# HKUST-Aerial-Robotics/FUEL

Hardware: NVIDIA H100
Metric: replans_per_sec (higher is better)
Workload: dtype f64 (cost/gradient), i32+f32 (ESDF), u8 (frontier)

## Files before the change

### fuel_b200/csrc/frontier.cu

```cuda
#include "common.cuh"

#include <cooperative_groups.h>

#include <algorithm>
#include <vector>

namespace cg = cooperative_groups;

namespace {

constexpr int NONE = 0x7fffffff;

struct FParams {
  int dom_lo[3], dom_n[3];
  int s_lo[3], s_hi[3];
  int z_min_idx;
  int cluster_min;
  double size_xy;
  float leaf, leaf_inv;
};

__device__ __forceinline__ int tri_at(const Geom& g, const uint8_t* __restrict__ occ, int x, int y,
                                      int z) {
  if (x < 0 || y < 0 || z < 0 || x >= g.nx || y >= g.ny || z >= g.nz) return -1;
// ... 1036 lines not shown
  int* c_final;
  int* ccur;
  int* cnext;
};

__global__ void stat_accum_kernel(Geom g, const int* __restrict__ k_addr, const int* __restrict__ k_cl,
                                  const ClusterMeta* __restrict__ meta, ClusterStat* st, LevelCtl ctl) {
  if (*ctl.n_new == 0) return;
  stat_accum_item(g, k_addr, k_cl, meta, st, *ctl.K, blockIdx.x * blockDim.x + threadIdx.x);
}

__global__ void downsample_kernel(Geom g, FParams fp, const int* __restrict__ k_addr,
                                  const int* __restrict__ k_cl, const int* __restrict__ cellidx,
                                  const ClusterMeta* __restrict__ meta, ClusterStat* st,
                                  float* __restrict__ k_cent, int* __restrict__ k_leaf, LevelCtl ctl) {
  if (*ctl.n_new == 0) return;
  downsample_item<true>(g, fp, k_addr, k_cl, cellidx, meta, st, k_cent, k_leaf, *ctl.K, blockIdx.x * blockDim.x + threadIdx.x);
}

__global__ void cov_kernel(Geom g, const int* __restrict__ k_cl, const int* __restrict__ k_leaf,
                           const float* __restrict__ k_cent, const ClusterMeta* __restrict__ meta,
                           ClusterStat* st, LevelCtl ctl) {
  if (*ctl.n_new == 0) return;
  cov_item<true>(g, k_cl, k_leaf, k_cent, meta, st, *ctl.K, blockIdx.x * blockDim.x + threadIdx.x);
}

__global__ void pca_kernel(Geom g, ClusterMeta* meta, const ClusterStat* __restrict__ st, LevelCtl ctl) {
  if (*ctl.n_new == 0) return;
  const int c = blockIdx.x * blockDim.x + threadIdx.x;
  mean_item(g, meta, st, *ctl.ccur, c);
  pca_item(meta, st, *ctl.ccur, c);
}

__global__ void side_count_kernel(Geom g, const int* __restrict__ k_addr, const int* __restrict__ k_cl,
                                  const ClusterMeta* __restrict__ meta, ClusterStat* st, LevelCtl ctl) {
  if (*ctl.n_new == 0) return;
  side_count_item(g, k_addr, k_cl, meta, st, *ctl.K, blockIdx.x * blockDim.x + threadIdx.x);
}

__global__ void __launch_bounds__(1024) split_alloc_kernel(ClusterMeta* meta, const ClusterStat* __restrict__ st,
                                                           LevelCtl ctl) {
  if (*ctl.n_new == 0) return;
  const int C = *ctl.ccur;
  __shared__ int made;
  split_alloc(meta, st, C, &made);
  __syncthreads();
  if (threadIdx.x == 0) {
    *ctl.cnext = C + made;
    *ctl.c_final = C + made;
    *ctl.n_new = made;
  }
}

__global__ void relabel_kernel(Geom g, const int* __restrict__ k_addr, int* __restrict__ k_cl,
                               const ClusterMeta* __restrict__ meta, LevelCtl ctl) {
  if (*ctl.n_new == 0) return;
  relabel_item(g, k_addr, k_cl, meta, *ctl.K, *ctl.ccur, blockIdx.x * blockDim.x + threadIdx.x);
}

__global__ void next_level_kernel(ClusterMeta* meta, ClusterStat* st, LevelCtl ctl) {
  if (*ctl.n_new == 0) return;
  const int c = blockIdx.x * blockDim.x + threadIdx.x;
  clear_do_split_item(meta, *ctl.ccur, c);
  stat_reset_item(st, meta, *ctl.cnext, c);
}

__global__ void init_meta_kernel(ClusterMeta* meta, ClusterStat* st, LevelCtl ctl) {
  const int R = *ctl.R;
  const int c = blockIdx.x * blockDim.x + threadIdx.x;
  init_meta_item(meta, R, c);
  stat_reset_item(st, meta, R, c);
  if (c == 0) {
    *ctl.ccur = R;
    *ctl.c_final = R;
    *ctl.n_new = (R > 0 && *ctl.K > 0) ? 1 : 0;
  }
}


constexpr int SMALL_CTAS = 8;
constexpr int SMALL_CAP = 32768;
constexpr int SMALL_CCAP = 8192;
constexpr int RES_K0 = 12288, RES_C0 = 256;


__device__ __forceinline__ void mark_chunk_item(const int* __restrict__ seed, const int* __restrict__ csize, int cluster_min,
                                                int* __restrict__ root_mask, int* __restrict__ kept_mask, int n, int i) {
  bool kept = false, root = false;
  if (i < n) {
    const int s = seed[i];
    kept = s != NONE && csize[s] > cluster_min;
    root = kept && s == i;
  }
  const unsigned mk = __ballot_sync(0xffffffffu, kept), mr = __ballot_sync(0xffffffffu, root);
  if ((i & 31) == 0 && i < n) {
    kept_mask[i >> 5] = (int)mk;
    root_mask[i >> 5] = (int)mr;
  }
}
__device__ void chunk_scan_small(const int* __restrict__ root_mask, const int* __restrict__ kept_mask,
                                 int* __restrict__ root_off, int* __restrict__ kept_off, int nchunk,
                                 int* __restrict__ tot_root, int* __restrict__ tot_kept) {
  __shared__ unsigned wtot2[32];
  const int t = threadIdx.x, lane = t & 31, w = t >> 5;
  const unsigned v = t < nchunk ? ((unsigned)__popc((unsigned)root_mask[t]) << 16) + (unsigned)__popc((unsigned)kept_mask[t]) : 0u;
  unsigned inc = v;
#pragma unroll
  for (int o = 1; o < 32; o <<= 1) {
    const unsigned u = __shfl_up_sync(0xffffffffu, inc, o);
    if (lane >= o) inc += u;
  }
  if (lane == 31) wtot2[w] = inc;
  __syncthreads();
  if (w == 0) {
    const unsigned x = wtot2[lane];
    unsigned xi = x;
#pragma unroll
    for (int o = 1; o < 32; o <<= 1) {
      const unsigned u = __shfl_up_sync(0xffffffffu, xi, o);
      if (lane >= o) xi += u;
    }
    wtot2[lane] = xi - x;
    if (lane == 31) {
      *tot_root = (int)(xi >> 16);
      *tot_kept = (int)(xi & 0xffffu);
    }
  }
  __syncthreads();
  if (t < nchunk) {
    const unsigned ex = wtot2[w] + inc - v;
    root_off[t] = (int)(ex >> 16);
    kept_off[t] = (int)(ex & 0xffffu);
  }
}
__device__ __forceinline__ void gather_chunk_item(const int* __restrict__ cell_addr, const int* __restrict__ seed,
                                                  const int* __restrict__ kept_mask, const int* __restrict__ kept_off,
                                                  const int* __restrict__ root_mask, const int* __restrict__ root_off,
                                                  int* __restrict__ k_addr, int* __restrict__ k_cl,
                                                  int* __restrict__ cellidx, int n, int i) {
  if (i >= n) return;
  const unsigned mk = (unsigned)kept_mask[i >> 5];
  const int a = cell_addr[i];
  if ((mk >> (i & 31)) & 1u) {
    const int k = kept_off[i >> 5] + __popc(mk & ((1u << (i & 31)) - 1u));
    const int s = seed[i];
    k_addr[k] = a;
    k_cl[k] = root_off[s >> 5] + __popc((unsigned)root_mask[s >> 5] & ((1u << (s & 31)) - 1u));
    cellidx[a] = k;
  } else {
    cellidx[a] = -1;
  }
}

struct SmallBufs {
  int *cell_addr, *parent, *claim, *csize, *seed, *is_root, *is_kept, *root_rank, *kept_off;
  uint8_t* cell_cls;
  int *k_addr, *k_cl, *k_leaf;
  float* k_cent;
  ClusterMeta* meta;
  ClusterStat* stat;
  int* counters;
  int* r_counters;
  ClusterMeta* r_meta;
  ClusterStat* r_stat;
  int *r_addr, *r_cl, *r_leaf;
  float* r_cent;
  int r_K, r_C;
};

__global__ void __cluster_dims__(SMALL_CTAS, 1, 1) __launch_bounds__(1024) cluster_small_kernel(Geom g, FParams fp, int8_t* __restrict__ flag,
                                                             int* __restrict__ cellidx, SmallBufs b) {
  cg::cluster_group cluster = cg::this_cluster();
  const int rank = (int)cluster.block_rank();
  const int tid = (((int)threadIdx.x >> 5) * SMALL_CTAS + rank) * 32 + ((int)threadIdx.x & 31);
  constexpr int NT = 1024 * SMALL_CTAS;
  const int n = b.counters[0];
#ifdef FUEL_PROF
  long long* prof = (long long*)(b.counters + 8);
  int pi = 0;
#define STAMP() do { if (tid == 0) { long long t_; asm volatile("mov.u64 %0, %%globaltimer;" : "=l"(t_)); prof[pi++] = t_; } } while (0)
#else
#define STAMP() do {} while (0)
#endif
  STAMP();
  if (n > SMALL_CAP) {
    if (tid == 0) {
      b.counters[4] = 1;
      b.r_counters[0] = n;
      b.r_counters[4] = 1;
    }
    return;
  }
#define FOR_ITEMS(i, N) for (int i = tid; i - tid < (N); i += NT)
  FOR_ITEMS(i, n) init_parent_item(b.parent, b.claim, b.csize, n, i);
  cluster.sync();
  STAMP();
  FOR_ITEMS(i, n) union_item(g, b.cell_addr, b.cell_cls, cellidx, b.parent, n, i);
  cluster.sync();
  STAMP();
  FOR_ITEMS(i, n) flatten_item(b.parent, b.cell_cls, n, i);
  cluster.sync();
  STAMP();
  FOR_ITEMS(i, n) claim_item(g, fp, b.cell_addr, b.cell_cls, cellidx, b.parent, b.claim, n, i);
  cluster.sync();
  STAMP();
  FOR_ITEMS(i, n) assign_item(b.cell_addr, b.cell_cls, b.parent, b.claim, b.seed, b.csize, flag, n, i);
  cluster.sync();
  STAMP();
  FOR_ITEMS(i, n) mark_chunk_item(b.seed, b.csize, fp.cluster_min, b.is_root, b.is_kept, n, i);
  cluster.sync();
  STAMP();
  if (rank == 0) chunk_scan_small(b.is_root, b.is_kept, b.root_rank, b.kept_off, (n + 31) >> 5, b.counters + 1, b.counters + 2);
  cluster.sync();
  STAMP();
  const int R = b.counters[1], K = b.counters[2];
  int C = R;
  int status = 0;
  if (R > 0 && K > 0) {
    FOR_ITEMS(i, n) gather_chunk_item(b.cell_addr, b.seed, b.is_kept, b.kept_off, b.is_root, b.root_rank, b.k_addr, b.k_cl,
                                      cellidx, n, i);
    FOR_ITEMS(c, R) {
      init_meta_item(b.meta, R, c);
      stat_reset_item(b.stat, b.meta, R, c);
    }
    cluster.sync();
    STAMP();
    for (int level = 0; level < 40; ++level) {
      if (2 * C > SMALL_CCAP) {
        status = 2;
        break;
      }
      FOR_ITEMS(k, K) stat_accum_item(g, b.k_addr, b.k_cl, b.meta, b.stat, K, k);
      cluster.sync();
      STAMP();
      FOR_ITEMS(c, C) mean_item(g, b.meta, b.stat, C, c);
      FOR_ITEMS(k, K) downsample_item<true>(g, fp, b.k_addr, b.k_cl, cellidx, b.meta, b.stat, b.k_cent, b.k_leaf, K, k);
      cluster.sync();
      STAMP();
      FOR_ITEMS(k, K) cov_item(g, b.k_cl, b.k_leaf, b.k_cent, b.meta, b.stat, K, k);
      cluster.sync();
      STAMP();
      FOR_ITEMS(c, C) pca_item(b.meta, b.stat, C, c);
      cluster.sync();
      STAMP();
      FOR_ITEMS(k, K) side_count_item(g, b.k_addr, b.k_cl, b.meta, b.stat, K, k);
      cluster.sync();
      STAMP();
      if (rank == 0) split_alloc(b.meta, b.stat, C, b.counters + 3);
      cluster.sync();
      STAMP();
      FOR_ITEMS(k, K) relabel_item(g, b.k_addr, b.k_cl, b.meta, K, C, k);
      cluster.sync();
      STAMP();
      const int n_new = b.counters[3];
      if (n_new == 0) break;
      FOR_ITEMS(c, C) clear_do_split_item(b.meta, C, c);
      C += n_new;
      FOR_ITEMS(c, C) stat_reset_item(b.stat, b.meta, C, c);
      cluster.sync();
      STAMP();
    }
  }
  FOR_ITEMS(i, n) reset_cellidx_item(b.cell_addr, cellidx, n, i);
  if (status == 0 && R > 0 && K > 0) {
    const int kp = min(K, b.r_K), cp = min(C, b.r_C);
    FOR_ITEMS(k, kp) {
      if (k < kp) {
        b.r_addr[k] = b.k_addr[k];
        b.r_cl[k] = b.k_cl[k];
        b.r_leaf[k] = b.k_leaf[k];
        b.r_cent[3 * k] = b.k_cent[3 * k];
        b.r_cent[3 * k + 1] = b.k_cent[3 * k + 1];
        b.r_cent[3 * k + 2] = b.k_cent[3 * k + 2];
      }
    }
    FOR_ITEMS(c, cp) {
      if (c < cp) {
        b.r_meta[c] = b.meta[c];
        b.r_stat[c] = b.stat[c];
      }
    }
  }
  if (tid == 0) {
    b.counters[4] = status;
    b.counters[5] = C;
    const int out[8] = { n, R, K, b.counters[3], status, C, b.counters[6], b.counters[7] };
#pragma unroll
    for (int j = 0; j < 8; ++j) b.r_counters[j] = out[j];
  }
#undef FOR_ITEMS
}

__global__ void is_changed_kernel(Geom g, const uint8_t* __restrict__ occ, const int* __restrict__ offs,
                                  const int* __restrict__ addr, uint8_t* __restrict__ changed, int* __restrict__ counts,
                                  int m) {
  const int c = blockIdx.x;
  if (c >= m) return;
  __shared__ int cnt;
  if (threadIdx.x == 0) cnt = 0;
  __syncthreads();
  int mine = 0;
  for (int i = offs[c] + threadIdx.x; i < offs[c + 1]; i += blockDim.x) {
    int x, y, z;
    addr_to_idx(g, addr[i], x, y, z);
    if (!frontier_pred(g, occ, x, y, z)) ++mine;
  }
  if (mine) atomicAdd(&cnt, mine);
  __syncthreads();
  if (threadIdx.x == 0) {
    if (changed) changed[c] = (uint8_t)(cnt > 0);
    if (counts) counts[c] = cnt;
  }
}

template <typename T>
struct DevBuf {
  T* p = nullptr;
  size_t cap = 0;
  int ensure(size_t n) {
    if (n <= cap) return 0;
    if (p) cudaFree(p);
    p = nullptr;
    cap = 0;
    size_t want = n + n / 4 + 1024;
    if (cudaMalloc(&p, want * sizeof(T)) != cudaSuccess) return FUELGPU_ENOMEM;
    cap = want;
    return 0;
  }
  int grow_preserve(size_t n, size_t keep, cudaStream_t s) {
    if (n <= cap) return 0;
    T* np = nullptr;
    size_t want = n + n / 2 + 1024;
    if (cudaMalloc(&np, want * sizeof(T)) != cudaSuccess) return FUELGPU_ENOMEM;
    if (p && keep) {
      cudaMemcpyAsync(np, p, keep * sizeof(T), cudaMemcpyDeviceToDevice, s);
      cudaStreamSynchronize(s);
    }
    if (p) cudaFree(p);
    p = np;
    cap = want;
    return 0;
  }
  void release() {
    if (p) cudaFree(p);
    p = nullptr;
    cap = 0;
  }
};

}

struct SweepPlan {
  bool words = false;
  unsigned nb = 0;
  size_t nmask = 0;
  int64_t ndom = 0;
  WordGeom wg;
};

struct HostView {
  const int *addr, *cl, *leaf;
  const float* cent;
  const ClusterMeta* meta;
  const ClusterStat* stat;
};

struct FrontierState {
  int* cellidx = nullptr;
  DevBuf<uint32_t> maskE, maskS;
  DevBuf<int> blockcnt, blockoff, scan_tot, scan_off;
  DevBuf<int> cell_addr, parent, claim, csize, seed, is_root, is_kept, root_rank, kept_off;
  DevBuf<uint8_t> cell_cls;
  DevBuf<int> k_addr, k_cl, k_leaf;
  DevBuf<float> k_cent;
  DevBuf<ClusterStat> stat;
  DevBuf<ClusterMeta> meta;
  DevBuf<char> res;
  bool small_ready = false;
  bool pend_active = false, pend_empty = true;
  FParams pend_fp;
  SweepPlan pend_plan;
  HostView pend_hv;
  cudaStream_t stream = nullptr;
  cudaEvent_t ev_in = nullptr;
  cudaEvent_t ev_out = nullptr;
  bool ev_out_valid = false;
  char* h_pin = nullptr;
  size_t h_pin_bytes = 0;
  int* d_counters = nullptr;
  std::vector<int32_t> h_cell_off, h_cell_addr, h_filt_off;
  std::vector<double> h_filtered, h_avg, h_bmin, h_bmax;
  int cell_order = FUELGPU_CELLS_BY_ADDRESS;
  float last_leaf = 0.f;
};

cudaStream_t frontier_stream_raw(FuelMap* m) { return m->fs->stream; }
cudaStream_t frontier_stream(FuelMap* m) {
  FrontierState* f = m->fs;
  cudaEventRecord(f->ev_in, m->stream);
  cudaStreamWaitEvent(f->stream, f->ev_in, 0);
  return f->stream;
}

int frontier_set_cell_order(FuelMap* m, int order) {
  if (order != FUELGPU_CELLS_BY_ADDRESS && order != FUELGPU_CELLS_BFS)
    return fuel_fail(m, FUELGPU_EINVAL, "unknown cell order");
  m->fs->cell_order = order;
  return 0;
}

void frontier_order_writer(FuelMap* m) {
  FrontierState* f = m->fs;
  if (f && f->ev_out_valid) cudaStreamWaitEvent(m->stream, f->ev_out, 0);
}

int frontier_state_create(FuelMap* m) {
  m->fs = new FrontierState();
  FUEL_CUDA(m, cudaStreamCreateWithFlags(&m->fs->stream, cudaStreamNonBlocking));
  FUEL_CUDA(m, cudaEventCreateWithFlags(&m->fs->ev_in, cudaEventDisableTiming));
  FUEL_CUDA(m, cudaEventCreateWithFlags(&m->fs->ev_out, cudaEventDisableTiming));
  FUEL_CUDA(m, cudaMalloc(&m->fs->cellidx, sizeof(int) * m->nvox));
  FUEL_CUDA(m, cudaMemsetAsync(m->fs->cellidx, 0xff, sizeof(int) * m->nvox, m->stream));
  FUEL_CUDA(m, cudaMalloc(&m->fs->d_counters, sizeof(int) * 8 + sizeof(long long) * 256));
  FUEL_CUDA(m, cudaMemsetAsync(m->fs->d_counters, 0, sizeof(int) * 8 + sizeof(long long) * 256, m->stream));
  return 0;
}

void frontier_state_destroy(FuelMap* m) {
  if (!m->fs) return;
  FrontierState* f = m->fs;
  if (f->cellidx) cudaFree(f->cellidx);
  if (f->d_counters) cudaFree(f->d_counters);
  if (f->h_pin) cudaFreeHost(f->h_pin);
  if (f->stream) {
    cudaStreamSynchronize(f->stream);
    cudaStreamDestroy(f->stream);
  }
  if (f->ev_in) cudaEventDestroy(f->ev_in);
  if (f->ev_out) cudaEventDestroy(f->ev_out);
  f->maskE.release(); f->maskS.release(); f->blockcnt.release(); f->blockoff.release();
  f->scan_tot.release(); f->scan_off.release();
  f->cell_addr.release(); f->parent.release(); f->claim.release(); f->csize.release();
  f->seed.release(); f->is_root.release(); f->is_kept.release(); f->root_rank.release();
  f->kept_off.release(); f->cell_cls.release(); f->k_addr.release(); f->k_cl.release();
  f->k_leaf.release(); f->k_cent.release(); f->stat.release(); f->meta.release(); f->res.release();
  delete f;
  m->fs = nullptr;
}

#define ENSURE(buf, n)                                         \
  do {                                                         \
    if ((buf).ensure(n)) return fuel_fail(m, FUELGPU_ENOMEM, "frontier: device allocation failed"); \
  } while (0)

static inline unsigned nblk(int64_t n, int b) { return (unsigned)((n + b - 1) / b); }

static int scan_ints(FuelMap* m, const int* in, int* out, int n, int* total) {
  FrontierState* f = m->fs;
  cudaStream_t s = m->fs->stream;
  if (n <= 4096) {
    scan_kernel<<<1, 1024, 0, s>>>(in, out, n, total);
    FUEL_LAUNCHES(m, 1);
    return 0;
  }
  const int nchunk = (n + 1023) / 1024;
  if (f->scan_tot.ensure(nchunk) || f->scan_off.ensure(nchunk))
    return fuel_fail(m, FUELGPU_ENOMEM, "frontier: device allocation failed");
  scan_chunks_kernel<<<nchunk, 1024, 0, s>>>(in, out, n, f->scan_tot.p);
  scan_kernel<<<1, 1024, 0, s>>>(f->scan_tot.p, f->scan_off.p, nchunk, total);
  scan_add_kernel<<<nchunk, 1024, 0, s>>>(out, n, f->scan_off.p);
  FUEL_LAUNCHES(m, 3);
  return 0;
}

static SweepPlan sweep_plan(const Geom& g, const FParams& fp) {
  SweepPlan pl;
  pl.ndom = (int64_t)fp.dom_n[0] * fp.dom_n[1] * fp.dom_n[2];
  pl.words = (g.nz % 32) == 0 && pl.ndom > 0;
  if (pl.words) {
    const int z0 = fp.dom_lo[2], z1 = fp.dom_lo[2] + fp.dom_n[2] - 1;
    pl.wg.wz0 = z0 >> 5;
    pl.wg.NW = (z1 >> 5) - pl.wg.wz0 + 1;
    pl.wg.nwords = (int64_t)fp.dom_n[0] * fp.dom_n[1] * pl.wg.NW;
    pl.nb = nblk(pl.wg.nwords, WORD_BLOCK);
    pl.nmask = (size_t)pl.nb * WORD_BLOCK;
  } else {
    pl.nb = nblk(pl.ndom, CLS_BLOCK);
    pl.nmask = (size_t)pl.nb * (CLS_BLOCK / 32);
  }
  return pl;
}

static int sweep_classify(FuelMap* m, const FParams& fp, const SweepPlan& pl, cudaStream_t s) {
  FrontierState* f = m->fs;
  ENSURE(f->maskE, pl.nmask);
  ENSURE(f->maskS, pl.nmask);
  ENSURE(f->blockcnt, pl.nb);
  ENSURE(f->blockoff, pl.nb);
  if (pl.words)
    classify_words_kernel<<<pl.nb, WORD_BLOCK, 0, s>>>(m->g, fp, pl.wg, m->occ, m->flag, f->maskE.p, f->maskS.p,
                                                       f->blockcnt.p);
  else
    classify_kernel<<<pl.nb, CLS_BLOCK, 0, s>>>(m->g, fp, m->occ, m->flag, f->maskE.p, f->maskS.p, f->blockcnt.p,
                                                pl.ndom);
  FUEL_LAUNCHES(m, 1);
  if (scan_ints(m, f->blockcnt.p, f->blockoff.p, (int)pl.nb, f->d_counters + 0)) return FUELGPU_ENOMEM;
  return 0;
}

static void sweep_compact(FuelMap* m, const FParams& fp, const SweepPlan& pl, int* cellidx, int cap, cudaStream_t s) {
  FrontierState* f = m->fs;
  if (pl.words)
    compact_words_kernel<<<pl.nb, WORD_BLOCK, 0, s>>>(m->g, fp, pl.wg, f->maskE.p, f->maskS.p, f->blockoff.p,
                                                      f->cell_addr.p, f->cell_cls.p, cellidx, cap);
  else
    compact_kernel<<<pl.nb, CLS_BLOCK, 0, s>>>(m->g, fp, f->maskE.p, f->maskS.p, f->blockoff.p, f->cell_addr.p,
                                               f->cell_cls.p, cellidx, pl.ndom, cap);
  FUEL_LAUNCHES(m, 1);
}

static size_t view_bytes(int K, int C) {
  return (size_t)K * (3 * sizeof(int) + 3 * sizeof(float)) + (size_t)C * (sizeof(ClusterMeta) + sizeof(ClusterStat)) + 64;
}

static int ensure_pin(FuelMap* m, size_t bytes) {
  FrontierState* f = m->fs;
  if (bytes <= f->h_pin_bytes) return 0;
  if (f->h_pin) cudaFreeHost(f->h_pin);
  f->h_pin = nullptr;
  f->h_pin_bytes = 0;
  FUEL_CUDA(m, cudaMallocHost((void**)&f->h_pin, bytes));
  f->h_pin_bytes = bytes;
  return 0;
}

struct ResultLayout {
  size_t meta, stat, addr, cl, leaf, cent, bytes;
};
static ResultLayout result_layout(int K, int C) {
  ResultLayout l;
  size_t p = 0;
  auto put = [&](size_t bytes) {
// ... 135 lines not shown
      for (int i = 0; i < cn; ++i) {
        int ijk[3];
        for (int a = 0; a < 3; ++a) ijk[a] = (int)(floorf(pf[(size_t)3 * i + a] * inv) - (float)minb[a]);
        lk[i] = std::make_pair(ijk[0] + ijk[1] * divb[0] + ijk[2] * divb[0] * divb[1], i);
      }
      std::sort(lk.begin(), lk.end());
      int nf = 0;
      for (int i = 0; i < cn;) {
        int j = i;
        float acc[3] = { 0.f, 0.f, 0.f };
        while (j < cn && lk[j].first == lk[i].first) {
          for (int a = 0; a < 3; ++a) acc[a] += pf[(size_t)3 * lk[j].second + a];
          ++j;
        }
        const float cntf = (float)(j - i);
        for (int a = 0; a < 3; ++a) new_filtered.push_back((double)(acc[a] / cntf));
        ++nf;
        i = j;
      }
      new_filt_off[r + 1] = new_filt_off[r] + nf;
    }
    r0 = r1;
  }
  f->h_filt_off.swap(new_filt_off);
  f->h_filtered.swap(new_filtered);
}

static int frontier_marshal(FuelMap* m, int K, int C, int32_t* n_clusters, int32_t* n_cells,
                            int32_t* n_filtered) {
  int rc = ensure_pin(m, view_bytes(K, C));
  if (rc) return rc;
  HostView hv;
  rc = enqueue_download(m, K, C, m->fs->h_pin, &hv);
  if (rc) return rc;
  FUEL_CUDA(m, cudaStreamSynchronize(m->fs->stream));
  return frontier_build_csr(m, K, C, hv, n_clusters, n_cells, n_filtered);
}

static int frontier_build_csr(FuelMap* m, int K, int C, const HostView& hv, int32_t* n_clusters,
                              int32_t* n_cells, int32_t* n_filtered) {
  FrontierState* f = m->fs;
  const Geom& g = m->g;
  const int* h_addr = hv.addr;
  const int* h_cl = hv.cl;
  const int* h_leaf = hv.leaf;
  const float* h_cent = hv.cent;
  const ClusterMeta* h_meta = hv.meta;
  const ClusterStat* h_stat = hv.stat;
  std::vector<int> order(C);
  for (int c = 0; c < C; ++c) order[c] = c;
  std::sort(order.begin(), order.end(), [&](int a, int b) {
    if (h_meta[a].root != h_meta[b].root) return h_meta[a].root < h_meta[b].root;
    return h_meta[a].path < h_meta[b].path;
  });
  std::vector<int> rank(C);
  for (int i = 0; i < C; ++i) rank[order[i]] = i;

  f->h_cell_off.assign(C + 1, 0);
  f->h_filt_off.assign(C + 1, 0);
  for (int k = 0; k < K; ++k) {
    f->h_cell_off[rank[h_cl[k]] + 1]++;
    if (h_leaf[k] >= 0) f->h_filt_off[rank[h_cl[k]] + 1]++;
  }
  for (int c = 0; c < C; ++c) {
    f->h_cell_off[c + 1] += f->h_cell_off[c];
    f->h_filt_off[c + 1] += f->h_filt_off[c];
  }
  f->h_cell_addr.resize(K);
  const int NF = f->h_filt_off[C];
  std::vector<std::pair<int, int>> filt_keys(NF);
  {
    std::vector<int> cur(f->h_cell_off.begin(), f->h_cell_off.end() - 1);
    std::vector<int> curf(f->h_filt_off.begin(), f->h_filt_off.end() - 1);
    for (int k = 0; k < K; ++k) {
      const int r = rank[h_cl[k]];
      f->h_cell_addr[cur[r]++] = h_addr[k];
      if (h_leaf[k] >= 0) filt_keys[curf[r]++] = std::make_pair(h_leaf[k], k);
    }
  }
  f->h_filtered.resize((size_t)3 * NF);
  for (int c = 0; c < C; ++c) {
    std::sort(filt_keys.begin() + f->h_filt_off[c], filt_keys.begin() + f->h_filt_off[c + 1]);
    for (int i = f->h_filt_off[c]; i < f->h_filt_off[c + 1]; ++i) {
      const int k = filt_keys[i].second;
      for (int a = 0; a < 3; ++a) f->h_filtered[(size_t)3 * i + a] = (double)h_cent[(size_t)3 * k + a];
    }
  }
  f->h_avg.resize((size_t)3 * C);
  f->h_bmin.resize((size_t)3 * C);
  f->h_bmax.resize((size_t)3 * C);
  for (int c = 0; c < C; ++c) {
    const int r = rank[c];
    for (int a = 0; a < 3; ++a) {
      f->h_avg[(size_t)3 * r + a] = h_meta[c].mean[a];
      f->h_bmin[(size_t)3 * r + a] = (h_stat[c].lo[a] + 0.5) * g.res + g.origin[a];
      f->h_bmax[(size_t)3 * r + a] = (h_stat[c].hi[a] + 0.5) * g.res + g.origin[a];
    }
  }
  *n_clusters = C;
  *n_cells = K;
  *n_filtered = NF;
  if (f->cell_order == FUELGPU_CELLS_BFS) {
    std::vector<int> out_root(C);
    for (int c = 0; c < C; ++c) out_root[rank[c]] = h_meta[c].root;
    frontier_apply_bfs_order(m, out_root);
    *n_filtered = f->h_filt_off[C];
  }
  return 0;
}

static int frontier_cluster_large(FuelMap* m, const FParams& fp, int n_cand, int32_t* n_clusters, int32_t* n_cells,
                                  int32_t* n_filtered);

static void frontier_make_params(FuelMap* m, const double umin[3], const double umax[3], const FuelFrontierParams* p,
                                 FParams* out) {
  FrontierState* f = m->fs;
  const Geom& g = m->g;
  const int nmax[3] = { g.nx, g.ny, g.nz };
  FParams fp;
  const double infl[3] = { 1, 1, 0.5 };
  for (int k = 0; k < 3; ++k) {
    double lo = umin[k] - infl[k], hi = umax[k] + infl[k];
    lo = lo > g.box_mind[k] ? lo : g.box_mind[k];
    hi = hi < g.box_maxd[k] ? hi : g.box_maxd[k];
    int ilo = (int)floor((lo - g.origin[k]) * g.res_inv);
    int ihi = (int)floor((hi - g.origin[k]) * g.res_inv);
    fp.s_lo[k] = ilo < 0 ? 0 : ilo;
    fp.s_hi[k] = ihi > nmax[k] - 1 ? nmax[k] - 1 : ihi;
    int dlo = g.box_min[k] < fp.s_lo[k] ? g.box_min[k] : fp.s_lo[k];
    int dhi = g.box_max[k] > fp.s_hi[k] ? g.box_max[k] : fp.s_hi[k];
    dlo = dlo < 0 ? 0 : dlo;
    dhi = dhi > nmax[k] - 1 ? nmax[k] - 1 : dhi;
    fp.dom_lo[k] = dlo;
    fp.dom_n[k] = dhi - dlo + 1;
    if (fp.dom_n[k] <= 0) {
      fp.dom_n[k] = 0;
    }
  }
  {
    int zi = 0;
    while (zi < g.nz && ((zi + 0.5) * g.res + g.origin[2]) < p->min_z) ++zi;
    fp.z_min_idx = zi;
  }
  fp.cluster_min = p->cluster_min;
  fp.size_xy = p->cluster_size_xy;
  fp.leaf = (float)(g.res * p->down_sample);
  f->last_leaf = fp.leaf;
  fp.leaf_inv = 1.0f / fp.leaf;
  f->pend_fp = fp;
  *out = fp;
}

static void frontier_clear_results(FrontierState* f) {
  f->h_cell_off.assign(1, 0);
  f->h_cell_addr.clear();
  f->h_filt_off.assign(1, 0);
  f->h_filtered.clear();
  f->h_avg.clear();
  f->h_bmin.clear();
  f->h_bmax.clear();
  f->pend_active = false;
  f->pend_empty = true;
}

int frontier_search_begin_impl(FuelMap* m, const double umin[3], const double umax[3],
                               const FuelFrontierParams* p) {
  FrontierState* f = m->fs;
  const Geom& g = m->g;
  cudaStream_t s = m->fs->stream;
  FParams fp;
  frontier_make_params(m, umin, umax, p, &fp);

  f->h_cell_off.assign(1, 0);
  f->h_cell_addr.clear();
  f->h_filt_off.assign(1, 0);
  f->h_filtered.clear();
  f->h_avg.clear();
  f->h_bmin.clear();
  f->h_bmax.clear();
  f->pend_active = false;
  f->pend_empty = true;

  const SweepPlan pl = sweep_plan(g, fp);
  if (pl.ndom <= 0) return 0;
  f->pend_empty = false;
  {
    const int rc = sweep_classify(m, fp, pl, s);
    if (rc) return rc;
  }
  {
    ENSURE(f->cell_addr, SMALL_CAP); ENSURE(f->cell_cls, SMALL_CAP); ENSURE(f->parent, SMALL_CAP);
    ENSURE(f->claim, SMALL_CAP); ENSURE(f->csize, SMALL_CAP); ENSURE(f->seed, SMALL_CAP);
    ENSURE(f->is_root, SMALL_CAP); ENSURE(f->is_kept, SMALL_CAP); ENSURE(f->root_rank, SMALL_CAP);
    ENSURE(f->kept_off, SMALL_CAP); ENSURE(f->k_addr, SMALL_CAP); ENSURE(f->k_cl, SMALL_CAP);
    ENSURE(f->k_leaf, SMALL_CAP); ENSURE(f->k_cent, (size_t)3 * SMALL_CAP);
    ENSURE(f->meta, SMALL_CCAP); ENSURE(f->stat, SMALL_CCAP);
    const ResultLayout rl = result_layout(RES_K0, RES_C0);
    ENSURE(f->res, 64 + rl.bytes);
    sweep_compact(m, fp, pl, f->cellidx, SMALL_CAP, s);
    SmallBufs sb;
    sb.cell_addr = f->cell_addr.p; sb.parent = f->parent.p; sb.claim = f->claim.p; sb.csize = f->csize.p;
    sb.seed = f->seed.p; sb.is_root = f->is_root.p; sb.is_kept = f->is_kept.p; sb.root_rank = f->root_rank.p;
    sb.kept_off = f->kept_off.p; sb.cell_cls = f->cell_cls.p; sb.k_addr = f->k_addr.p; sb.k_cl = f->k_cl.p;
    sb.k_leaf = f->k_leaf.p; sb.k_cent = f->k_cent.p; sb.meta = f->meta.p; sb.stat = f->stat.p;
    sb.counters = f->d_counters;
    {
      char* rb = f->res.p + 64;
      sb.r_counters = (int*)f->res.p;
      sb.r_meta = (ClusterMeta*)(rb + rl.meta); sb.r_stat = (ClusterStat*)(rb + rl.stat);
      sb.r_addr = (int*)(rb + rl.addr); sb.r_cl = (int*)(rb + rl.cl); sb.r_leaf = (int*)(rb + rl.leaf);
      sb.r_cent = (float*)(rb + rl.cent);
      sb.r_K = RES_K0;
      sb.r_C = RES_C0;
    }
    cluster_small_kernel<<<SMALL_CTAS, 1024, 0, s>>>(g, fp, m->flag, f->cellidx, sb);
    FUEL_LAUNCHES(m, 1);
    int rc0 = ensure_pin(m, 64 + rl.bytes);
    if (rc0) return rc0;
    FUEL_CUDA(m, cudaMemcpyAsync(f->h_pin, f->res.p, 64 + rl.bytes, cudaMemcpyDeviceToHost, s));
    result_view(rl, f->h_pin + 64, &f->pend_hv);
    f->pend_fp = fp;
    f->pend_plan = pl;
    f->pend_active = true;
  }
  cudaEventRecord(f->ev_out, f->stream);
  f->ev_out_valid = true;
  return 0;
}

int frontier_search_end_impl(FuelMap* m, int32_t* n_clusters, int32_t* n_cells, int32_t* n_filtered) {
  FrontierState* f = m->fs;
  const Geom& g = m->g;
  cudaStream_t s = m->fs->stream;
  *n_clusters = *n_cells = *n_filtered = 0;
  if (f->pend_empty || !f->pend_active) {
    f->pend_active = false;
    return 0;
  }
  f->pend_active = false;
  const FParams fp = f->pend_fp;
  const SweepPlan pl = f->pend_plan;
  int n_cand = 0;
  {
    const int* cnt = (const int*)f->h_pin;
    HostView& hv = f->pend_hv;
    FUEL_CUDA(m, cudaStreamSynchronize(s));
    n_cand = cnt[0];
    if (n_cand == 0) return 0;
    if (cnt[4] == 0) {
      const int R = cnt[1], K = cnt[2], C = cnt[5];
      if (R == 0 || K == 0) return 0;
      if (K <= RES_K0 && C <= RES_C0) return frontier_build_csr(m, K, C, hv, n_clusters, n_cells, n_filtered);
      return frontier_marshal(m, K, C, n_clusters, n_cells, n_filtered);
    }
    if (cnt[4] == 1) {
      reset_cellidx_kernel<<<nblk(SMALL_CAP, 256), 256, 0, s>>>(f->cell_addr.p, f->cellidx, SMALL_CAP);
      FUEL_LAUNCHES(m, 1);
    }
  }

  ENSURE(f->cell_addr, n_cand); ENSURE(f->cell_cls, n_cand); ENSURE(f->parent, n_cand);
  ENSURE(f->claim, n_cand); ENSURE(f->csize, n_cand); ENSURE(f->seed, n_cand);
  ENSURE(f->is_root, n_cand); ENSURE(f->is_kept, n_cand); ENSURE(f->root_rank, n_cand);
  ENSURE(f->kept_off, n_cand);

  sweep_compact(m, fp, pl, f->cellidx, n_cand, s);
  return frontier_cluster_large(m, fp, n_cand, n_clusters, n_cells, n_filtered);
}

static int frontier_cluster_large(FuelMap* m, const FParams& fp, int n_cand, int32_t* n_clusters, int32_t* n_cells,
                                  int32_t* n_filtered) {
  FrontierState* f = m->fs;
  const Geom& g = m->g;
  cudaStream_t s = m->fs->stream;
  ENSURE(f->parent, n_cand);
  ENSURE(f->claim, n_cand); ENSURE(f->csize, n_cand); ENSURE(f->seed, n_cand);
  ENSURE(f->is_root, n_cand); ENSURE(f->is_kept, n_cand); ENSURE(f->root_rank, n_cand);
  ENSURE(f->kept_off, n_cand);
  ENSURE(f->k_addr, n_cand); ENSURE(f->k_cl, n_cand); ENSURE(f->k_leaf, n_cand); ENSURE(f->k_cent, (size_t)3 * n_cand);
  ENSURE(f->meta, (size_t)n_cand + 1024);
  ENSURE(f->stat, (size_t)n_cand + 1024);
  const unsigned cb = nblk(n_cand, 256);
  init_parent_kernel<<<cb, 256, 0, s>>>(f->parent.p, f->claim.p, f->csize.p, n_cand);
  union_kernel<<<cb, 256, 0, s>>>(g, f->cell_addr.p, f->cell_cls.p, f->cellidx, f->parent.p, n_cand);
  flatten_kernel<<<cb, 256, 0, s>>>(f->parent.p, f->cell_cls.p, n_cand);
  claim_kernel<<<cb, 256, 0, s>>>(g, fp, f->cell_addr.p, f->cell_cls.p, f->cellidx, f->parent.p, f->claim.p, n_cand);
  assign_kernel<<<cb, 256, 0, s>>>(f->cell_addr.p, f->cell_cls.p, f->parent.p, f->claim.p, f->seed.p,
                                   f->csize.p, m->flag, n_cand);
  mark_kernel<<<cb, 256, 0, s>>>(f->seed.p, f->csize.p, fp.cluster_min, f->is_root.p, f->is_kept.p, n_cand);
  FUEL_LAUNCHES(m, 6);
  if (scan_ints(m, f->is_root.p, f->root_rank.p, n_cand, f->d_counters + 1)) return FUELGPU_ENOMEM;
  if (scan_ints(m, f->is_kept.p, f->kept_off.p, n_cand, f->d_counters + 2)) return FUELGPU_ENOMEM;
  gather_kept_kernel<<<cb, 256, 0, s>>>(f->cell_addr.p, f->seed.p, f->is_kept.p, f->kept_off.p,
                                        f->root_rank.p, f->k_addr.p, f->k_cl.p, f->cellidx, n_cand);
  FUEL_LAUNCHES(m, 1);

  LevelCtl ctl;
  ctl.R = f->d_counters + 1;
  ctl.K = f->d_counters + 2;
  ctl.n_new = f->d_counters + 3;
  ctl.c_final = f->d_counters + 5;
  ctl.ccur = f->d_counters + 6;
  ctl.cnext = f->d_counters + 7;
  const int64_t r_ub = n_cand / ((fp.cluster_min > 0 ? fp.cluster_min : 0) + 1) + 1;
  init_meta_kernel<<<nblk(r_ub, 256), 256, 0, s>>>(f->meta.p, f->stat.p, ctl);
  FUEL_LAUNCHES(m, 1);
  int cnt[8] = { 0, 0, 0, 0, 0, 0, 0, 0 };
  constexpr int LEVELS_PER_BATCH = 12, MAX_LEVELS = 36;
  auto c_bound = [&](int level) -> int64_t {
    const int64_t c = level < 24 ? (r_ub << level) : (int64_t)n_cand;
    return c > n_cand ? (int64_t)n_cand : c;
  };
  for (int level = 0; level < MAX_LEVELS; ++level) {
    const unsigned ccb = nblk(c_bound(level), 256);
    stat_accum_kernel<<<cb, 256, 0, s>>>(g, f->k_addr.p, f->k_cl.p, f->meta.p, f->stat.p, ctl);
    downsample_kernel<<<cb, 256, 0, s>>>(g, fp, f->k_addr.p, f->k_cl.p, f->cellidx, f->meta.p, f->stat.p,
                                         f->k_cent.p, f->k_leaf.p, ctl);
    cov_kernel<<<cb, 256, 0, s>>>(g, f->k_cl.p, f->k_leaf.p, f->k_cent.p, f->meta.p, f->stat.p, ctl);
    pca_kernel<<<ccb, 256, 0, s>>>(g, f->meta.p, f->stat.p, ctl);
    side_count_kernel<<<cb, 256, 0, s>>>(g, f->k_addr.p, f->k_cl.p, f->meta.p, f->stat.p, ctl);
    split_alloc_kernel<<<1, 1024, 0, s>>>(f->meta.p, f->stat.p, ctl);
    relabel_kernel<<<cb, 256, 0, s>>>(g, f->k_addr.p, f->k_cl.p, f->meta.p, ctl);
    next_level_kernel<<<nblk(c_bound(level + 1), 256), 256, 0, s>>>(f->meta.p, f->stat.p, ctl);
    FUEL_LAUNCHES(m, 8);
    int* t = ctl.ccur;
    ctl.ccur = ctl.cnext;
    ctl.cnext = t;
    if ((level + 1) % LEVELS_PER_BATCH == 0 || level + 1 == MAX_LEVELS) {
      FUEL_CUDA(m, cudaMemcpyAsync(cnt, f->d_counters, sizeof(int) * 8, cudaMemcpyDeviceToHost, s));
      FUEL_CUDA(m, cudaStreamSynchronize(s));
      if (cnt[3] == 0) break;
    }
  }
  reset_cellidx_kernel<<<cb, 256, 0, s>>>(f->cell_addr.p, f->cellidx, n_cand);
  FUEL_LAUNCHES(m, 1);
  FUEL_CUDA(m, cudaGetLastError());
  const int R = cnt[1], K = cnt[2], C = cnt[5];
  if (R == 0 || K == 0) return 0;
  return frontier_marshal(m, K, C, n_clusters, n_cells, n_filtered);
}


__global__ void set_cellidx_kernel(const int* __restrict__ cell_addr, int* __restrict__ cellidx, int n) {
  const int i = blockIdx.x * blockDim.x + threadIdx.x;
  if (i < n) cellidx[cell_addr[i]] = i;
}

int frontier_candidates_impl(FuelMap* m, const double umin[3], const double umax[3], const FuelFrontierParams* p, int z_lo,
                             int z_hi, int32_t* n_out) {
  FrontierState* f = m->fs;
  const Geom& g = m->g;
  cudaStream_t s = frontier_stream(m);
  FParams fp;
  frontier_make_params(m, umin, umax, p, &fp);
  *n_out = 0;
  const int dz0 = fp.dom_lo[2] > z_lo ? fp.dom_lo[2] : z_lo;
  const int dz1 = (fp.dom_lo[2] + fp.dom_n[2] - 1) < z_hi ? (fp.dom_lo[2] + fp.dom_n[2] - 1) : z_hi;
  if (dz1 < dz0) return 0;
  fp.dom_lo[2] = dz0;
  fp.dom_n[2] = dz1 - dz0 + 1;
  const SweepPlan pl = sweep_plan(g, fp);
  if (pl.ndom <= 0) return 0;
  {
    const int rc = sweep_classify(m, fp, pl, s);
    if (rc) return rc;
  }
  int n = 0;
  FUEL_CUDA(m, cudaMemcpyAsync(&n, f->d_counters, sizeof(int), cudaMemcpyDeviceToHost, s));
  FUEL_CUDA(m, cudaStreamSynchronize(s));
  if (n > 0) {
    ENSURE(f->cell_addr, n);
    ENSURE(f->cell_cls, n);
    sweep_compact(m, fp, pl, nullptr, n, s);
    FUEL_CUDA(m, cudaGetLastError());
  }
  *n_out = n;
  return 0;
}

int frontier_candidates_fetch_impl(FuelMap* m, int32_t n, int32_t* addr, uint8_t* cls) {
  FrontierState* f = m->fs;
  if (n <= 0) return 0;
  cudaStream_t s = f->stream;
  FUEL_CUDA(m, cudaMemcpyAsync(addr, f->cell_addr.p, sizeof(int) * n, cudaMemcpyDeviceToHost, s));
  FUEL_CUDA(m, cudaMemcpyAsync(cls, f->cell_cls.p, n, cudaMemcpyDeviceToHost, s));
  FUEL_CUDA(m, cudaStreamSynchronize(s));
  return 0;
}

int frontier_search_from_candidates_impl(FuelMap* m, const double umin[3], const double umax[3], const FuelFrontierParams* p,
                                         int32_t n, const int32_t* addr, const uint8_t* cls, int32_t* n_clusters,
                                         int32_t* n_cells, int32_t* n_filtered) {
  FrontierState* f = m->fs;
  cudaStream_t s = frontier_stream(m);
  FParams fp;
  frontier_make_params(m, umin, umax, p, &fp);
  frontier_clear_results(f);
  *n_clusters = *n_cells = *n_filtered = 0;
  if (n <= 0) return 0;
  for (int i = 1; i < n; ++i)
    if (addr[i] <= addr[i - 1]) return fuel_fail(m, FUELGPU_EINVAL, "candidate addresses must be strictly ascending");
  if (addr[0] < 0 || (int64_t)addr[n - 1] >= m->nvox) return fuel_fail(m, FUELGPU_EINVAL, "candidate address outside the map");
  ENSURE(f->cell_addr, n);
  ENSURE(f->cell_cls, n);
  FUEL_CUDA(m, cudaMemcpyAsync(f->cell_addr.p, addr, sizeof(int) * n, cudaMemcpyHostToDevice, s));
  FUEL_CUDA(m, cudaMemcpyAsync(f->cell_cls.p, cls, n, cudaMemcpyHostToDevice, s));
  set_cellidx_kernel<<<nblk(n, 256), 256, 0, s>>>(f->cell_addr.p, f->cellidx, n);
  FUEL_LAUNCHES(m, 1);
  FUEL_CUDA(m, cudaMemcpyAsync(f->d_counters, &n, sizeof(int), cudaMemcpyHostToDevice, s));
  const int rc = frontier_cluster_large(m, fp, n, n_clusters, n_cells, n_filtered);
  cudaEventRecord(f->ev_out, f->stream);
  f->ev_out_valid = true;
  return rc;
}

int frontier_search_impl(FuelMap* m, const double umin[3], const double umax[3],
                         const FuelFrontierParams* p, int32_t* n_clusters, int32_t* n_cells,
                         int32_t* n_filtered) {
  int rc = frontier_search_begin_impl(m, umin, umax, p);
  if (rc) return rc;
  return frontier_search_end_impl(m, n_clusters, n_cells, n_filtered);
}

int frontier_fetch_impl(FuelMap* m, int32_t* cell_offsets, int32_t* cell_addr, int32_t* filt_offsets,
                        double* filtered, double* average, double* box_min, double* box_max) {
  FrontierState* f = m->fs;
  if (cell_offsets) memcpy(cell_offsets, f->h_cell_off.data(), sizeof(int32_t) * f->h_cell_off.size());
  if (cell_addr) memcpy(cell_addr, f->h_cell_addr.data(), sizeof(int32_t) * f->h_cell_addr.size());
  if (filt_offsets) memcpy(filt_offsets, f->h_filt_off.data(), sizeof(int32_t) * f->h_filt_off.size());
  if (filtered) memcpy(filtered, f->h_filtered.data(), sizeof(double) * f->h_filtered.size());
  if (average) memcpy(average, f->h_avg.data(), sizeof(double) * f->h_avg.size());
  if (box_min) memcpy(box_min, f->h_bmin.data(), sizeof(double) * f->h_bmin.size());
  if (box_max) memcpy(box_max, f->h_bmax.data(), sizeof(double) * f->h_bmax.size());
  return 0;
}

int ensure_fr_scratch(FuelMap* m, size_t bytes) {
  if (bytes <= m->fr_scr_bytes) return 0;
  if (m->fr_scr) {
    cudaDeviceSynchronize();
    cudaFree(m->fr_scr);
  }
  m->fr_scr = nullptr;
  m->fr_scr_bytes = 0;
  const size_t want = bytes + bytes / 2 + 4096;
  FUEL_CUDA(m, cudaMalloc(&m->fr_scr, want));
  m->fr_scr_bytes = want;
  return 0;
}

int frontier_is_changed_impl(FuelMap* m, int32_t mcl, const int32_t* offs, const int32_t* addr,
                             uint8_t* changed, int32_t* counts) {
  if (mcl <= 0) return 0;
  const int ncell = offs[mcl];
  const size_t nci = (size_t)(ncell > 0 ? ncell : 1);
  int rc = ensure_fr_scratch(m, sizeof(int) * ((size_t)2 * mcl + 1 + nci) + mcl + 16);
  if (rc) return rc;
  int* d_off = (int*)m->fr_scr;
  int* d_addr = d_off + mcl + 1;
  int* d_cnt = d_addr + nci;
  uint8_t* d_ch = (uint8_t*)(d_cnt + mcl);
  cudaStream_t s = m->fs->stream;
  FUEL_CUDA(m, cudaMemcpyAsync(d_off, offs, sizeof(int) * (mcl + 1), cudaMemcpyHostToDevice, s));
  if (ncell > 0) FUEL_CUDA(m, cudaMemcpyAsync(d_addr, addr, sizeof(int) * ncell, cudaMemcpyHostToDevice, s));
  is_changed_kernel<<<mcl, 128, 0, s>>>(m->g, m->occ, d_off, d_addr, d_ch, d_cnt, mcl);
  FUEL_LAUNCHES(m, 1);
  if (changed) FUEL_CUDA(m, cudaMemcpyAsync(changed, d_ch, mcl, cudaMemcpyDeviceToHost, s));
  if (counts) FUEL_CUDA(m, cudaMemcpyAsync(counts, d_cnt, sizeof(int) * mcl, cudaMemcpyDeviceToHost, s));
  FUEL_CUDA(m, cudaStreamSynchronize(s));
  return 0;
}

#ifdef FUEL_PROF
extern "C" __attribute__((visibility("default"))) int fuelgpu_debug_frontier_prof(FuelMap* m, long long* out,
                                                                                  int n) {
  cudaMemcpy(out, (long long*)(m->fs->d_counters + 8), sizeof(long long) * n, cudaMemcpyDeviceToHost);
  return 0;
}
#endif
```

Measured before the change: 2008.

## Build ordered frontier CSR result on device instead of host

Moves the per-replan CSR construction (cluster ranking by root/path key, cell grouping, leaf-sorted filtered centroids, offsets and bounding boxes) from host code into the tail of the small cluster kernel. It runs on CTA rank 0 using shared-memory radix split passes, and writes into a fixed ResultBlock that is copied to pinned memory, so the host only memcpys at fetch time. This removes host-side sorting and marshalling from the replan loop. In exchange it adds serial single-CTA GPU work at the end of the kernel. The fast path only applies for the by-address cell order.

```diff
diff --git a/fuel_b200/csrc/frontier.cu b/fuel_b200/csrc/frontier.cu
--- a/fuel_b200/csrc/frontier.cu
+++ b/fuel_b200/csrc/frontier.cu
@@ -1212,6 +1212,14 @@
   }
 }
 
+struct ResultBlock {
+  int counters[16];
+  int cell_off[RES_C0 + 1], filt_off[RES_C0 + 1];
+  double avg[RES_C0][3], bmin[RES_C0][3], bmax[RES_C0][3];
+  int cell_addr[RES_K0];
+  float filtered[RES_K0][3];
+};
+
 struct SmallBufs {
   int *cell_addr, *parent, *claim, *csize, *seed, *is_root, *is_kept, *root_rank, *kept_off;
   uint8_t* cell_cls;
@@ -1220,13 +1228,159 @@
   ClusterMeta* meta;
   ClusterStat* stat;
   int* counters;
-  int* r_counters;
-  ClusterMeta* r_meta;
-  ClusterStat* r_stat;
-  int *r_addr, *r_cl, *r_leaf;
-  float* r_cent;
-  int r_K, r_C;
+  ResultBlock* res;
 };
+
+constexpr int ORD_WARPS = 32, ORD_ROUNDS = RES_K0 / (ORD_WARPS * 32);
+static_assert(ORD_ROUNDS * ORD_WARPS * 32 == RES_K0, "a warp's run of RES_K0 items is a whole number of rounds");
+static_assert(RES_C0 <= 256, "a cluster's output rank is one digit");
+static_assert(RES_K0 <= (1 << 14), "a kept index takes the low 14 bits of a list entry");
+
+struct OrderSmem {
+  int hist[ORD_WARPS][256];
+  int start[257];
+  unsigned long long key[RES_C0];
+  int rank[RES_C0];
+  int wsum[8];
+  int max_leaf, n_list;
+};
+
+__device__ __forceinline__ void scan_256(OrderSmem& sm, int* v) {
+  const int t = threadIdx.x, lane = t & 31, w = t >> 5;
+  int x = 0, inc = 0;
+  if (t < 256) {
+    x = inc = v[t];
+#pragma unroll
+    for (int o = 1; o < 32; o <<= 1) {
+      const int u = __shfl_up_sync(0xffffffffu, inc, o);
+      if (lane >= o) inc += u;
+    }
+    if (lane == 31) sm.wsum[w] = inc;
+  }
+  __syncthreads();
+  if (t < 256) {
+    int off = 0;
+    for (int u = 0; u < w; ++u) off += sm.wsum[u];
+    v[t] = off + inc - x;
+    if (t == 255) v[256] = off + inc;
+  }
+  __syncthreads();
+}
+
+template <class DigitF, class EmitF>
+__device__ __forceinline__ void split_pass(OrderSmem& sm, int n, DigitF digit, EmitF emit) {
+  const int t = threadIdx.x, lane = t & 31, w = t >> 5;
+  const int per = (n + ORD_WARPS * 32 - 1) / (ORD_WARPS * 32) * 32;
+  const int base = w * per;
+  for (int d = lane; d < 256; d += 32) sm.hist[w][d] = 0;
+  __syncwarp();
+  int dg[ORD_ROUNDS];
+#pragma unroll
+  for (int r = 0; r < ORD_ROUNDS; ++r) {
+    const int i = base + r * 32 + lane;
+    dg[r] = (r * 32 < per && i < n) ? digit(i) : -1;
+  }
+#pragma unroll
+  for (int r = 0; r < ORD_ROUNDS; ++r) {
+    if (r * 32 < per) {
+      const unsigned peers = __match_any_sync(0xffffffffu, dg[r]);
+      if (dg[r] >= 0 && lane == __ffs(peers) - 1) sm.hist[w][dg[r]] += __popc(peers);
+      __syncwarp();
+    }
+  }
+  __syncthreads();
+  if (t < 256) {
+    int run = 0;
+    for (int v = 0; v < ORD_WARPS; ++v) {
+      const int c = sm.hist[v][t];
+      sm.hist[v][t] = run;
+      run += c;
+    }
+    sm.start[t] = run;
+  }
+  __syncthreads();
+  scan_256(sm, sm.start);
+#pragma unroll
+  for (int r = 0; r < ORD_ROUNDS; ++r) {
+    if (r * 32 < per) {
+      const int d = dg[r];
+      const unsigned peers = __match_any_sync(0xffffffffu, d);
+      if (d >= 0) emit(sm.start[d] + sm.hist[w][d] + __popc(peers & ((1u << lane) - 1u)), base + r * 32 + lane);
+      __syncwarp();
+      if (d >= 0 && lane == __ffs(peers) - 1) sm.hist[w][d] += __popc(peers);
+      __syncwarp();
+    }
+  }
+  __syncthreads();
+}
+
+struct OrderIn {
+  const int *k_addr, *k_cl, *k_leaf;
+  const float* k_cent;
+  const ClusterMeta* meta;
+  const ClusterStat* stat;
+  double res, origin[3];
+};
+
+__device__ __noinline__ void order_result(OrderIn b, ResultBlock* res, int K, int C, unsigned long long* list0,
+                                          unsigned long long* list1) {
+  __shared__ OrderSmem sm;
+  const int t = threadIdx.x;
+  if (t < C) sm.key[t] = ((unsigned long long)(unsigned)b.meta[t].root << 32) | b.meta[t].path;
+  if (t == 0) sm.max_leaf = sm.n_list = 0;
+  __syncthreads();
+  if (t < C) {
+    const unsigned long long key = sm.key[t];
+    int r = 0;
+    for (int c = 0; c < C; ++c) r += sm.key[c] < key;
+    sm.rank[t] = r;
+    for (int a = 0; a < 3; ++a) {
+      res->avg[r][a] = b.meta[t].mean[a];
+      res->bmin[r][a] = (b.stat[t].lo[a] + 0.5) * b.res + b.origin[a];
+      res->bmax[r][a] = (b.stat[t].hi[a] + 0.5) * b.res + b.origin[a];
+    }
+  }
+  int ml = 0;
+  for (int k = t; k < K; k += 1024) ml = max(ml, b.k_leaf[k]);
+  ml = __reduce_max_sync(0xffffffffu, ml);
+  if ((t & 31) == 0) atomicMax(&sm.max_leaf, ml);
+  __syncthreads();
+
+  const int leaf_bits = 32 - __clz(sm.max_leaf), key_bits = leaf_bits + 32 - __clz(C - 1);
+  for (int k = t; k - t < K; k += 1024) {
+    const int leaf = k < K ? b.k_leaf[k] : -1;
+    const unsigned owners = __ballot_sync(0xffffffffu, leaf >= 0);
+    int at = 0;
+    if ((t & 31) == 0 && owners) at = atomicAdd(&sm.n_list, __popc(owners));
+    at = __shfl_sync(0xffffffffu, at, 0) + __popc(owners & ((1u << (t & 31)) - 1u));
+    if (leaf >= 0) {
+      const unsigned long long key = ((unsigned long long)sm.rank[b.k_cl[k]] << leaf_bits) | (unsigned)leaf;
+      list0[at] = (key << 14) | (unsigned)k;
+    }
+  }
+
+  split_pass(sm, K, [&](int k) { return sm.rank[b.k_cl[k]]; },
+             [&](int pos, int k) { res->cell_addr[pos] = b.k_addr[k]; });
+  if (t <= C) res->cell_off[t] = sm.start[t];
+
+  const int NF = sm.n_list;
+  unsigned long long *src = list0, *dst = list1;
+  for (int shift = 14; shift < 14 + key_bits; shift += 8) {
+    split_pass(sm, NF, [&](int i) { return (int)(src[i] >> shift) & 255; }, [&](int pos, int i) { dst[pos] = src[i]; });
+    unsigned long long* const x = src;
+    src = dst;
+    dst = x;
+  }
+  for (int i = t; i < NF; i += 1024) {
+    const int k = (int)(src[i] & 16383u);
+    for (int a = 0; a < 3; ++a) res->filtered[i][a] = b.k_cent[3 * k + a];
+    const int r = (int)(src[i] >> (14 + leaf_bits));
+    for (int q = i ? (int)(src[i - 1] >> (14 + leaf_bits)) + 1 : 0; q <= r; ++q) res->filt_off[q] = i;
+    if (i == NF - 1)
+      for (int q = r + 1; q <= C; ++q) res->filt_off[q] = NF;
+  }
+  if (t == 0) res->counters[8] = NF;
+}
 
 __global__ void __cluster_dims__(SMALL_CTAS, 1, 1) __launch_bounds__(1024) cluster_small_kernel(Geom g, FParams fp, int8_t* __restrict__ flag,
                                                              int* __restrict__ cellidx, SmallBufs b) {
@@ -1246,8 +1400,8 @@
   if (n > SMALL_CAP) {
     if (tid == 0) {
       b.counters[4] = 1;
-      b.r_counters[0] = n;
-      b.r_counters[4] = 1;
+      b.res->counters[0] = n;
+      b.res->counters[4] = 1;
     }
     return;
   }
@@ -1322,31 +1476,17 @@
     }
   }
   FOR_ITEMS(i, n) reset_cellidx_item(b.cell_addr, cellidx, n, i);
-  if (status == 0 && R > 0 && K > 0) {
-    const int kp = min(K, b.r_K), cp = min(C, b.r_C);
-    FOR_ITEMS(k, kp) {
-      if (k < kp) {
-        b.r_addr[k] = b.k_addr[k];
-        b.r_cl[k] = b.k_cl[k];
-        b.r_leaf[k] = b.k_leaf[k];
-        b.r_cent[3 * k] = b.k_cent[3 * k];
-        b.r_cent[3 * k + 1] = b.k_cent[3 * k + 1];
-        b.r_cent[3 * k + 2] = b.k_cent[3 * k + 2];
-      }
-    }
-    FOR_ITEMS(c, cp) {
-      if (c < cp) {
-        b.r_meta[c] = b.meta[c];
-        b.r_stat[c] = b.stat[c];
-      }
-    }
+  if (rank == 0 && status == 0 && R > 0 && K > 0 && K <= RES_K0 && C <= RES_C0) {
+    const OrderIn in = { b.k_addr, b.k_cl, b.k_leaf, b.k_cent, b.meta, b.stat, g.res, { g.origin[0], g.origin[1], g.origin[2] } };
+    order_result(in, b.res, K, C, (unsigned long long*)b.is_kept, (unsigned long long*)b.kept_off);
+    STAMP();
   }
   if (tid == 0) {
     b.counters[4] = status;
     b.counters[5] = C;
     const int out[8] = { n, R, K, b.counters[3], status, C, b.counters[6], b.counters[7] };
 #pragma unroll
-    for (int j = 0; j < 8; ++j) b.r_counters[j] = out[j];
+    for (int j = 0; j < 8; ++j) b.res->counters[j] = out[j];
   }
 #undef FOR_ITEMS
 }
@@ -1440,7 +1580,6 @@
   bool pend_active = false, pend_empty = true;
   FParams pend_fp;
   SweepPlan pend_plan;
-  HostView pend_hv;
   cudaStream_t stream = nullptr;
   cudaEvent_t ev_in = nullptr;
   cudaEvent_t ev_out = nullptr;
@@ -1448,6 +1587,7 @@
   char* h_pin = nullptr;
   size_t h_pin_bytes = 0;
   int* d_counters = nullptr;
+  const ResultBlock* h_res = nullptr;
   std::vector<int32_t> h_cell_off, h_cell_addr, h_filt_off;
   std::vector<double> h_filtered, h_avg, h_bmin, h_bmax;
   int cell_order = FUELGPU_CELLS_BY_ADDRESS;
@@ -1889,6 +2029,7 @@
 }
 
 static void frontier_clear_results(FrontierState* f) {
+  f->h_res = nullptr;
   f->h_cell_off.assign(1, 0);
   f->h_cell_addr.clear();
   f->h_filt_off.assign(1, 0);
@@ -1907,16 +2048,7 @@
   cudaStream_t s = m->fs->stream;
   FParams fp;
   frontier_make_params(m, umin, umax, p, &fp);
-
-  f->h_cell_off.assign(1, 0);
-  f->h_cell_addr.clear();
-  f->h_filt_off.assign(1, 0);
-  f->h_filtered.clear();
-  f->h_avg.clear();
-  f->h_bmin.clear();
-  f->h_bmax.clear();
-  f->pend_active = false;
-  f->pend_empty = true;
+  frontier_clear_results(f);
 
   const SweepPlan pl = sweep_plan(g, fp);
   if (pl.ndom <= 0) return 0;
@@ -1932,8 +2064,7 @@
     ENSURE(f->kept_off, SMALL_CAP); ENSURE(f->k_addr, SMALL_CAP); ENSURE(f->k_cl, SMALL_CAP);
     ENSURE(f->k_leaf, SMALL_CAP); ENSURE(f->k_cent, (size_t)3 * SMALL_CAP);
     ENSURE(f->meta, SMALL_CCAP); ENSURE(f->stat, SMALL_CCAP);
-    const ResultLayout rl = result_layout(RES_K0, RES_C0);
-    ENSURE(f->res, 64 + rl.bytes);
+    ENSURE(f->res, sizeof(ResultBlock));
     sweep_compact(m, fp, pl, f->cellidx, SMALL_CAP, s);
     SmallBufs sb;
     sb.cell_addr = f->cell_addr.p; sb.parent = f->parent.p; sb.claim = f->claim.p; sb.csize = f->csize.p;
@@ -1941,21 +2072,12 @@
     sb.kept_off = f->kept_off.p; sb.cell_cls = f->cell_cls.p; sb.k_addr = f->k_addr.p; sb.k_cl = f->k_cl.p;
     sb.k_leaf = f->k_leaf.p; sb.k_cent = f->k_cent.p; sb.meta = f->meta.p; sb.stat = f->stat.p;
     sb.counters = f->d_counters;
-    {
-      char* rb = f->res.p + 64;
-      sb.r_counters = (int*)f->res.p;
-      sb.r_meta = (ClusterMeta*)(rb + rl.meta); sb.r_stat = (ClusterStat*)(rb + rl.stat);
-      sb.r_addr = (int*)(rb + rl.addr); sb.r_cl = (int*)(rb + rl.cl); sb.r_leaf = (int*)(rb + rl.leaf);
-      sb.r_cent = (float*)(rb + rl.cent);
-      sb.r_K = RES_K0;
-      sb.r_C = RES_C0;
-    }
+    sb.res = (ResultBlock*)f->res.p;
     cluster_small_kernel<<<SMALL_CTAS, 1024, 0, s>>>(g, fp, m->flag, f->cellidx, sb);
     FUEL_LAUNCHES(m, 1);
-    int rc0 = ensure_pin(m, 64 + rl.bytes);
+    int rc0 = ensure_pin(m, sizeof(ResultBlock));
     if (rc0) return rc0;
-    FUEL_CUDA(m, cudaMemcpyAsync(f->h_pin, f->res.p, 64 + rl.bytes, cudaMemcpyDeviceToHost, s));
-    result_view(rl, f->h_pin + 64, &f->pend_hv);
+    FUEL_CUDA(m, cudaMemcpyAsync(f->h_pin, f->res.p, sizeof(ResultBlock), cudaMemcpyDeviceToHost, s));
     f->pend_fp = fp;
     f->pend_plan = pl;
     f->pend_active = true;
@@ -1979,15 +2101,21 @@
   const SweepPlan pl = f->pend_plan;
   int n_cand = 0;
   {
-    const int* cnt = (const int*)f->h_pin;
-    HostView& hv = f->pend_hv;
+    const ResultBlock* rb = (const ResultBlock*)f->h_pin;
+    const int* cnt = rb->counters;
     FUEL_CUDA(m, cudaStreamSynchronize(s));
     n_cand = cnt[0];
     if (n_cand == 0) return 0;
     if (cnt[4] == 0) {
       const int R = cnt[1], K = cnt[2], C = cnt[5];
       if (R == 0 || K == 0) return 0;
-      if (K <= RES_K0 && C <= RES_C0) return frontier_build_csr(m, K, C, hv, n_clusters, n_cells, n_filtered);
+      if (K <= RES_K0 && C <= RES_C0 && f->cell_order == FUELGPU_CELLS_BY_ADDRESS) {
+        f->h_res = rb;
+        *n_clusters = C;
+        *n_cells = K;
+        *n_filtered = cnt[8];
+        return 0;
+      }
       return frontier_marshal(m, K, C, n_clusters, n_cells, n_filtered);
     }
     if (cnt[4] == 1) {
@@ -2162,6 +2290,20 @@
 int frontier_fetch_impl(FuelMap* m, int32_t* cell_offsets, int32_t* cell_addr, int32_t* filt_offsets,
                         double* filtered, double* average, double* box_min, double* box_max) {
   FrontierState* f = m->fs;
+  if (const ResultBlock* rb = f->h_res) {
+    const size_t C = rb->counters[5], K = rb->counters[2], NF = rb->counters[8];
+    if (cell_offsets) memcpy(cell_offsets, rb->cell_off, sizeof(int32_t) * (C + 1));
+    if (cell_addr) memcpy(cell_addr, rb->cell_addr, sizeof(int32_t) * K);
+    if (filt_offsets) memcpy(filt_offsets, rb->filt_off, sizeof(int32_t) * (C + 1));
+    if (filtered) {
+      const float* cent = &rb->filtered[0][0];
+      for (size_t i = 0; i < 3 * NF; ++i) filtered[i] = (double)cent[i];
+    }
+    if (average) memcpy(average, rb->avg, sizeof(double) * 3 * C);
+    if (box_min) memcpy(box_min, rb->bmin, sizeof(double) * 3 * C);
+    if (box_max) memcpy(box_max, rb->bmax, sizeof(double) * 3 * C);
+    return 0;
+  }
   if (cell_offsets) memcpy(cell_offsets, f->h_cell_off.data(), sizeof(int32_t) * f->h_cell_off.size());
   if (cell_addr) memcpy(cell_addr, f->h_cell_addr.data(), sizeof(int32_t) * f->h_cell_addr.size());
   if (filt_offsets) memcpy(filt_offsets, f->h_filt_off.data(), sizeof(int32_t) * f->h_filt_off.size());
```

After: 2379, median of 6. +18.5%, better.
